# peach-xiao/EMRT

Measured on AMD Instinct MI355X. Metric: training tiles/sec at 256x256, higher is better.
Workload: dtype bf16; 1 GPU; EMRT ResNet50, Potsdam 256x256, 6 classes, batch 8 per GPU, fwd+bwd+SGD step (BASELINE configs[1]), bf16; global_batch=8, parallelism=dp1, hipgraph=True

## Files before the change

emrt_amd/csrc/common.hpp:

```cpp
#pragma once
#include <hip/hip_runtime.h>
#include <stdint.h>
#include <stdio.h>
#include <string.h>
#include "../../include/emrt_hip.h"

#define EMRT_F32 0
#define EMRT_BF16 1
#define EMRT_F16 2

namespace emrt {

extern thread_local char g_err[512];
inline int fail(const char* fn, const char* msg) {
  snprintf(g_err, sizeof(g_err), "%s: %s", fn, msg);
  return -1;
}
inline int check_launch(const char* fn) {
  hipError_t e = hipGetLastError();
  if (e != hipSuccess) {
    snprintf(g_err, sizeof(g_err), "%s: launch failed: %s", fn, hipGetErrorString(e));
    return -2;
  }
  return 0;
// ... 8 lines not shown
  int wgrad_split;
  int thin_cblk;
  int thin_blocks;
  int thin_ch;
  int no_thin_bwd;
  int igemm64_nst;
  int wgrad_nst;
  int pair_max;
  int msda_fwd_global;
  int msda_bwd_global;
  int msda_lds_min_pairs;
  int msda_bwd_dref_lds;
  int msda_band_halo;
  int msda_scatter_qsplit;
  int msda_scatter_cuts;
  int msda_fwd_chunks;
  int msda_fwd_threads;
  int msda_fwd_probe;
  int bn_block_kb;
  int bn_slice_c;
  int bn_operand_blocks;
  int ln_bwd_rows;
  int ln_bwd_max_blocks;
  int ln_bwd_threads;
  int ln_atomic;
  int gn_group_blocks;
  int gn_stat_rows;
  int gn_bwd_stat_rows;
  int gn_apply_rows;
  int igemm8p_probe;
  int igemm8p_cmajor;
  int igemm8p_min_blocks;
  int wgrad8p_min_steps;
  int wgrad8p_slab;
  int wgrad8p_xcd;
  int wgrad8p_force;
  int no_ksplit128;
  int wgrad_no_overwrite;
  int no_s2_dgrad;
  int wgroup_blocks;
  int wgroup_min_steps;
  int wgroup_max;
  int wgroup8;
  int wgroup8_blocks;
  int wgroup8_min_work;
  int msda_scatter_merge;
  int msda_scatter_mfma;
  int msda_mf_bands;
  int sgd_nt;
  int mha_bwd_split;
  int mha_valu;
  int no_bna;
  int memcpy_kernel;
  int xk;
};
extern Tuning g_tune;

struct Scratch {
  void* ptr; size_t bytes; void* stream;
  unsigned* tick;
  float* xk_part;
};
constexpr size_t SCRATCH_TICK_BYTES = 65536;
constexpr int SCRATCH_TICKS = (int)(SCRATCH_TICK_BYTES / 4);
constexpr size_t SCRATCH_XK_BYTES = 8u << 20;
extern Scratch g_scratch;

struct bf16_t {
  unsigned short v;
};
struct f16_t {
  unsigned short v;
};

__device__ __forceinline__ float to_f32(float x) { return x; }
__device__ __forceinline__ float to_f32(bf16_t x) { return __uint_as_float(((uint32_t)x.v) << 16); }
__device__ __forceinline__ float to_f32(f16_t x) { return (float)__builtin_bit_cast(_Float16, x.v); }
__device__ __forceinline__ float bf16_bits_to_f32(uint32_t lo16) { return __uint_as_float(lo16 << 16); }
__device__ __forceinline__ float f16_bits_to_f32(uint32_t lo16) { return (float)__builtin_bit_cast(_Float16, (unsigned short)lo16); }

template <class T>
__device__ __forceinline__ T from_f32(float f);
template <>
__device__ __forceinline__ float from_f32<float>(float f) {
  return f;
}
template <>
__device__ __forceinline__ bf16_t from_f32<bf16_t>(float f) {
  __bf16 b = (__bf16)f;
  bf16_t r;
  r.v = __builtin_bit_cast(unsigned short, b);
  return r;
}
template <>
__device__ __forceinline__ f16_t from_f32<f16_t>(float f) {
  f16_t r;
  r.v = __builtin_bit_cast(unsigned short, (_Float16)f);
  return r;
}
typedef __attribute__((ext_vector_type(2))) _Float16 emrt_half2_t;
typedef __attribute__((ext_vector_type(2))) float emrt_float2_t;
__device__ __forceinline__ uint32_t pack_f16x2(float lo, float hi) {
  emrt_half2_t h = __builtin_convertvector((emrt_float2_t){lo, hi}, emrt_half2_t);
  return __builtin_bit_cast(uint32_t, h);
}
__device__ __forceinline__ void unpack_f16x2(uint32_t w, float& lo, float& hi) {
// ... 249 lines not shown
```

emrt_amd/csrc/conv.hip:

```cpp
#include "common.hpp"
#include "bn_operand.hpp"
#include <stdlib.h>
#include <type_traits>

using namespace emrt;

typedef __attribute__((ext_vector_type(8))) __bf16 bf16x8_t;
typedef __attribute__((ext_vector_type(4))) short short4_t;
typedef __attribute__((ext_vector_type(16))) float f32x16_t;

struct ConvArgs {
  const void* in = nullptr;
  const void* w = nullptr;
  void* out = nullptr;
  const float* bias = nullptr;
  const float* scale = nullptr;
  const void* res = nullptr;
  int N = 0, H = 0, W = 0, C = 0, ldin = 0;
  long long in_bs = 0;
  int OH = 0, OW = 0, OC = 0, ldout = 0;
  long long out_bs = 0;
  int ldres = 0;
  long long res_bs = 0;
  int KH = 0, KW = 0, stride = 0, pad = 0;
// ... 1457 lines not shown
  const int gv = vec ? G : 1;
  const size_t lds = (size_t)gv * 2 * 2 * Cfg::BKM * Cfg::PITCH;
  static bool attr_done = false;
  if (!attr_done) {
    if (hipFuncSetAttribute(reinterpret_cast<const void*>(wgrad_kernel<T, true, G>), hipFuncAttributeMaxDynamicSharedMemorySize,
                            (int)((size_t)G * 4 * Cfg::BKM * Cfg::PITCH)) != hipSuccess ||
        hipFuncSetAttribute(reinterpret_cast<const void*>(wgrad_kernel<T, false, 1>), hipFuncAttributeMaxDynamicSharedMemorySize,
                            (int)((size_t)4 * Cfg::BKM * Cfg::PITCH)) != hipSuccess)
      return fail("emrt_conv2d_wgrad", "cannot raise the dynamic LDS limit");
    attr_done = true;
  }
  const int xcd = g_tune.wgrad8p_xcd;
  const unsigned grid1 = 8u * (unsigned)(((long long)tx * ty * S + 7) / 8);
  if (vec && g_tune.wgrad_nst == 3) {
    static bool attr3 = false;
    if (!attr3) { (void)hipFuncSetAttribute(reinterpret_cast<const void*>(wgrad_kernel<T, true, G, 3>), hipFuncAttributeMaxDynamicSharedMemorySize, (int)((size_t)G * 4 * Cfg::BKM * Cfg::PITCH)); attr3 = true; }
    hipLaunchKernelGGL((wgrad_kernel<T, true, G, 3>), dim3(grid1), dim3(256 * G), lds, st, a, tx, ty, S, xcd);
  } else if (vec) hipLaunchKernelGGL((wgrad_kernel<T, true, G>), dim3(grid1), dim3(256 * G), lds, st, a, tx, ty, S, xcd);
  else hipLaunchKernelGGL((wgrad_kernel<T, false, 1>), dim3(grid1), dim3(256), lds, st, a, tx, ty, S, xcd);
  return check_launch("emrt_conv2d_wgrad");
}

extern "C" int emrt_conv2d_wgrad(const void* x, const void* dy, float* dw,
                                 int N, int H, int W, int C, int ldx, long long x_bs,
                                 int OH, int OW, int OC, int lddy, long long dy_bs,
                                 int KH, int KW, int stride, int pad, float* dbias, int dilation, int dtype, void* stream) {
  EMRT_REQUIRE(x && dy && dw, "null pointer");
  const ConvShape s = {N, H, W, C, OH, OW, OC, KH, KW, stride, pad, dilation};
  EMRT_CONV_CHECK(s, ldx, x_bs, lddy, dy_bs, dtype, CK_DIMS);
  EMRT_REQUIRE(dilation >= 1, "bad dims");
  EMRT_CONV_CHECK(s, ldx, x_bs, lddy, dy_bs, dtype, CK_SIZE | CK_PIXELS);
  EMRT_REQUIRE_TRAIN_DTYPE(dtype);
  EMRT_CONV_CHECK(s, ldx, x_bs, lddy, dy_bs, dtype, CK_X | CK_Y | CK_X24);
  const WgradArgs a = wgrad_args(x, dy, dw, dbias, N, H, W, C, ldx, x_bs, OH, OW, OC, lddy, dy_bs, KH, KW, stride, pad, dilation, 0);
  hipStream_t st = (hipStream_t)stream;
  return with_train_dtype("emrt_conv2d_wgrad", dtype, [&](auto t) { return wgrad_dispatch<decltype(t)>(a, st); });
}

struct ThinBwdArgs {
  const void* x; const void* dy; const void* wd; void* dx; float* dw; float* dbias; double* stats; const void* mask_y;
  int HW, C, OC, ldx, lddy, lddx, ldy, accumulate, pix_per_block, cg_shift;
  float mask_scale;
  long long x_bs, dy_bs, dx_bs, y_bs, M;
  const float* bn_mean; const float* bn_invstd; const float* bn_gamma; const float* bn_beta;
};

template <class T, int CH>
struct VecN;
template <class T>
struct VecN<T, 4> : Vec4<T> {};
template <class T>
struct VecN<T, 8> : Vec8<T> {};

template <class T, int CH, int MASK, bool ACC, bool BNX = false>
__global__ __launch_bounds__(256, CH == 4 ? 4 : 2) void thin_bwd_kernel(ThinBwdArgs p) {
  constexpr int U = 2;
  using V = VecN<T, CH>;
  __shared__ float red[32 * 256];
  const T* x = (const T*)p.x;
  const T* dy = (const T*)p.dy;
  const T* wd = (const T*)p.wd;
  const T* ym = (const T*)p.mask_y;
  T* dx = (T*)p.dx;
  const int tid = threadIdx.x;
  const int CG = 1 << p.cg_shift, ppb = 256 >> p.cg_shift;
  const int cg = tid & (CG - 1), pl = tid >> p.cg_shift;
  const int c0 = (int)blockIdx.y * (CH << p.cg_shift) + cg * CH;
  const int lane = tid & 63;
  const int grp = CG < 64 ? CG : 64;
  const int gpos = lane & (grp - 1), gbase = lane - gpos;
  float w[8][CH], dwa[8][CH], ss[CH], sq[CH], db[8];
#pragma unroll
  for (int o = 0; o < 8; ++o) {
    db[o] = 0.f;
#pragma unroll
    for (int j = 0; j < CH; ++j) {
      w[o][j] = o < p.OC ? to_f32(wd[(c0 + j) * p.OC + o]) : 0.f;
      dwa[o][j] = 0.f;
    }
  }
#pragma unroll
  for (int j = 0; j < CH; ++j) { ss[j] = 0.f; sq[j] = 0.f; }
  float bsc[BNX ? CH : 1], bsh[BNX ? CH : 1];
  if (BNX) {
#pragma unroll
    for (int j = 0; j < CH; ++j) bn_scale_shift(p.bn_mean[c0 + j], p.bn_invstd[c0 + j], p.bn_gamma[c0 + j], p.bn_beta[c0 + j], bsc[j], bsh[j]);
  }
  const int xbs = (int)p.x_bs, dybs = (int)p.dy_bs, dxbs = (int)p.dx_bs, ybs = (int)p.y_bs, M = (int)p.M;
  const int m0 = (int)blockIdx.x * p.pix_per_block;
  const int m1 = m0 + p.pix_per_block < M ? m0 + p.pix_per_block : M;
  for (int mb = m0 + pl; mb < m1; mb += U * ppb) {
    float xv[U][CH], yv[U][CH], old[U][CH], mydy[U];
    bool ok[U];
    int oo[U];
#pragma unroll
    for (int u = 0; u < U; ++u) {
      const int m = mb + u * ppb;
      ok[u] = m < m1;
      mydy[u] = 0.f;
      if (!ok[u]) continue;
      const int nb = m / p.HW;
      const int pix = m - nb * p.HW;
      oo[u] = nb * dxbs + pix * p.lddx + c0;
      V::load(x + (nb * xbs + pix * p.ldx + c0), xv[u]);
      if (MASK == 2) V::load(ym + (nb * ybs + pix * p.ldy + c0), yv[u]);
      if (ACC) V::load(dx + oo[u], old[u]);
      if (gpos < p.OC) mydy[u] = to_f32(dy[nb * dybs + pix * p.lddy + gpos]);
    }
#pragma unroll
    for (int u = 0; u < U; ++u) {
      float dyv[8];
#pragma unroll
      for (int o = 0; o < 8; ++o) dyv[o] = __shfl(mydy[u], gbase + o, 64);
      if (!ok[u]) continue;
      if (BNX) {
#pragma unroll
        for (int j = 0; j < CH; ++j) xv[u][j] = fmaxf(fmaf(xv[u][j], bsc[j], bsh[j]), 0.f);
      }
      float v[CH];
#pragma unroll
      for (int j = 0; j < CH; ++j) {
        float a = 0.f;
#pragma unroll
        for (int o = 0; o < 8; ++o) a = fmaf(dyv[o], w[o][j], a);
        if (ACC) a += old[u][j];
        float second = 0.f;
        if (MASK) {
          second = MASK == 1 ? xv[u][j] : yv[u][j];
          a = second > 0.f ? a * p.mask_scale : 0.f;
        }
        v[j] = a;
        const float q = to_f32(from_f32<T>(a));
        ss[j] += q;
        sq[j] = fmaf(q, MASK ? second : q, sq[j]);
      }
      V::store(dx + oo[u], v);
#pragma unroll
      for (int o = 0; o < 8; ++o) {
#pragma unroll
        for (int j = 0; j < CH; ++j) dwa[o][j] = fmaf(dyv[o], xv[u][j], dwa[o][j]);
        if (cg == 0 && blockIdx.y == 0) db[o] += dyv[o];
      }
    }
  }
#pragma unroll
  for (int rnd = 0; rnd < CH / 4; ++rnd) {
    if (rnd * 32 >= p.OC * CH) break;
    if (rnd) __syncthreads();
#pragma unroll
    for (int k = 0; k < 32; ++k) red[k * 256 + tid] = dwa[(rnd * 32 + k) / CH][(rnd * 32 + k) % CH];
    __syncthreads();
    for (int k = pl; k < 32; k += ppb) {
      const int kk = rnd * 32 + k;
      if (kk >= p.OC * CH) break;
      float a = 0.f;
      for (int q = 0; q < ppb; ++q) a += red[k * 256 + q * CG + cg];
      atomicAdd(p.dw + (kk / CH) * p.C + c0 + (kk % CH), a);
    }
  }
  if (p.stats || p.dbias) {
    __syncthreads();
#pragma unroll
    for (int k = 0; k < CH; ++k) {
      red[k * 256 + tid] = ss[k];
      red[(CH + k) * 256 + tid] = sq[k];
    }
    if (cg == 0) {
#pragma unroll
      for (int k = 0; k < 8; ++k) red[(2 * CH + k) * 256 + pl] = db[k];
    }
    __syncthreads();
    if (p.stats) {
      double* rep = p.stats + (long long)(blockIdx.x & 7) * 2 * p.C;
      for (int k = pl; k < 2 * CH; k += ppb) {
        float a = 0.f;
        for (int q = 0; q < ppb; ++q) a += red[k * 256 + q * CG + cg];
        atomicAdd(rep + (k / CH) * p.C + c0 + (k % CH), (double)a);
      }
    }
    if (p.dbias && tid < p.OC) {
      float a = 0.f;
      for (int q = 0; q < ppb; ++q) a += red[(2 * CH + tid) * 256 + q];
      atomicAdd(p.dbias + tid, a);
    }
  }
}

template <class T>
static bool thin_bwd_ok(const ConvArgs& d, const WgradArgs& w) {
  constexpr int EPC = 4;
  const int C = w.C;
  if (w.KH != 1 || w.KW != 1 || w.stride != 1 || w.pad != 0 || w.OC > 8) return false;
  if (d.stat_x || (d.res && d.mask_y) || (d.res && d.res != d.out)) return false;
  if (C < 32 || C > 1024 || (C & (C - 1))) return false;
  const long long px = (long long)w.H * w.W - 1, LIM = 1ll << 31;
  if ((long long)w.N * w.H * w.W >= LIM || (w.N - 1) * w.x_bs + px * w.ldx + C >= LIM || (w.N - 1) * d.out_bs + px * d.ldout + C >= LIM ||
      (w.N - 1) * w.dy_bs + px * w.lddy + w.OC >= LIM || (d.mask_y && (w.N - 1) * d.y_bs + px * d.ldy + C >= LIM)) return false;
  auto al = [](const void* q) { return ((uintptr_t)q) % 16 == 0; };
  if (!al(w.x) || !al(d.out) || (d.mask_y && !al(d.mask_y))) return false;
  if (w.ldx % EPC || w.x_bs % EPC || d.ldout % EPC || d.out_bs % EPC) return false;
  if (d.mask_y && (d.ldy % EPC || d.y_bs % EPC)) return false;
  return true;
}

template <class T, int CH>
static int thin_bwd_launch_ch(const ConvArgs& d, const WgradArgs& w, hipStream_t st, const float* const* xbn = nullptr) {
  ThinBwdArgs a;
  a.x = w.x; a.dy = w.dy; a.wd = d.w; a.dx = d.out; a.dw = w.dw; a.dbias = w.dbias; a.stats = d.stats; a.mask_y = d.mask_y;
  a.HW = w.H * w.W; a.C = w.C; a.OC = w.OC; a.ldx = w.ldx; a.lddy = w.lddy; a.lddx = d.ldout; a.ldy = d.ldy;
  a.accumulate = d.res != nullptr;
  a.mask_scale = d.mask_scale;
  a.x_bs = w.x_bs; a.dy_bs = w.dy_bs; a.dx_bs = d.out_bs; a.y_bs = d.y_bs;
  a.M = (long long)w.N * w.H * w.W;
  int cblk = g_tune.thin_cblk;
  if (cblk < 8 * CH) cblk = 8 * CH;
  if (cblk > w.C) cblk = w.C;
  if (cblk > 256 * CH) cblk = 256 * CH;
  int sh = 0;
  while ((CH << sh) < cblk) ++sh;
  a.cg_shift = sh;
  const int cchunks = w.C / (CH << sh);
  const int ppb = 256 >> sh;
  const long long want_chunks = g_tune.thin_blocks > 0 ? g_tune.thin_blocks : 128;
  long long per = (a.M + want_chunks - 1) / want_chunks;
  per = (per + 2 * ppb - 1) / (2 * ppb) * (2 * ppb);
  if (per < 8 * ppb) per = 8 * ppb;
  a.pix_per_block = (int)per;
  const long long blocks = (a.M + per - 1) / per;
  const bool same = d.mask_y && d.mask_y == w.x && d.ldy == w.ldx && d.y_bs == w.x_bs;
  const int mask = !d.mask_y ? 0 : (same ? 1 : 2);
  const dim3 grid((unsigned)blocks, (unsigned)cchunks), block(256);
  a.bn_mean = a.bn_invstd = a.bn_gamma = a.bn_beta = nullptr;
  if (xbn) {
    if (mask != 1 || a.accumulate) return fail("emrt_bn_pointwise_bwd", "internal: the BatchNorm-operand form is the mask-from-input, overwrite form");
    a.bn_mean = xbn[0]; a.bn_invstd = xbn[1]; a.bn_gamma = xbn[2]; a.bn_beta = xbn[3];
    hipLaunchKernelGGL((thin_bwd_kernel<T, CH, 1, false, true>), grid, block, 0, st, a);
    return check_launch("emrt_bn_pointwise_bwd");
  }
  if (a.accumulate) {
    hipLaunchKernelGGL((thin_bwd_kernel<T, CH, 0, true>), grid, block, 0, st, a);
  } else if (mask == 0) {
    hipLaunchKernelGGL((thin_bwd_kernel<T, CH, 0, false>), grid, block, 0, st, a);
  } else if (mask == 1) {
    hipLaunchKernelGGL((thin_bwd_kernel<T, CH, 1, false>), grid, block, 0, st, a);
  } else {
    hipLaunchKernelGGL((thin_bwd_kernel<T, CH, 2, false>), grid, block, 0, st, a);
  }
  return check_launch("emrt_conv2d_bwd");
}

template <class T>
static int thin_bwd_launch(const ConvArgs& d, const WgradArgs& w, hipStream_t st, const float* const* xbn = nullptr) {
  const int want = g_tune.thin_ch;
  constexpr int EPC = 16 / (int)sizeof(T);
  const bool can8 = w.C >= 64 && w.ldx % 8 == 0 && w.x_bs % 8 == 0 && d.ldout % 8 == 0 && d.out_bs % 8 == 0 &&
                    (!d.mask_y || (d.ldy % 8 == 0 && d.y_bs % 8 == 0)) && EPC <= 8;
  if (want == 8 && can8) return thin_bwd_launch_ch<T, 8>(d, w, st, xbn);
  return thin_bwd_launch_ch<T, 4>(d, w, st, xbn);
}

struct ThinFwdArgs {
  const void* x; const void* w; const float* bias; void* out;
  int HW, C, OC, ldx, ldo;
  long long x_bs, o_bs, M;
};

template <class T>
struct Raw8;
template <>
struct Raw8<bf16_t> {
  uint4 q;
  __device__ __forceinline__ void load(const bf16_t* p) { q = *reinterpret_cast<const uint4*>(p); }
  __device__ __forceinline__ void unpack(float (&o)[8]) const { Vec8<bf16_t>::unpack(q, o); }
};
template <>
struct Raw8<float> {
  float4 a, b;
  __device__ __forceinline__ void load(const float* p) { a = *reinterpret_cast<const float4*>(p); b = *reinterpret_cast<const float4*>(p + 4); }
  __device__ __forceinline__ void unpack(float (&o)[8]) const { o[0] = a.x; o[1] = a.y; o[2] = a.z; o[3] = a.w; o[4] = b.x; o[5] = b.y; o[6] = b.z; o[7] = b.w; }
};

template <class T, int CGS>
__global__ __launch_bounds__(256, 2) void thin_fwd_bn_kernel(ThinFwdArgs p, BnOperand bn) {
  constexpr int CH = 8, U = 4;
  extern __shared__ float bn_lds[];
  const T* x = (const T*)p.x;
  const T* wp = (const T*)p.w;
  T* out = (T*)p.out;
  const int tid = threadIdx.x;
  constexpr int CG = 1 << CGS, ppb = 256 >> CGS;
  const int cg = tid & (CG - 1), pl = tid >> CGS;
  const int c0 = cg * CH;
  const int M = (int)p.M, HW = p.HW, xbs = (int)p.x_bs, obs = (int)p.o_bs;
  const int step = (int)gridDim.x * ppb * U;
  int mb = (int)blockIdx.x * ppb * U + pl;
  auto xoff = [&](int m) {
    const int mc = m < M ? m : 0;
    const int nb = mc / HW;
    return nb * xbs + (mc - nb * HW) * p.ldx + c0;
  };
  Raw8<T> xv[U], xn[U];
#pragma unroll
  for (int u = 0; u < U; ++u) xv[u].load(x + xoff(mb + u * ppb));
  bn_operand_preamble(bn, p.C, bn_lds, blockIdx.x == 0);
  float sc[CH], sh[CH], w[8][CH];
#pragma unroll
  for (int j = 0; j < CH; ++j) { sc[j] = bn_lds[c0 + j]; sh[j] = bn_lds[p.C + c0 + j]; }
#pragma unroll
  for (int o = 0; o < 8; ++o) {
    float wv[CH];
    Vec8<T>::load(wp + ((o < p.OC ? o : 0) * p.C + c0), wv);
#pragma unroll
    for (int j = 0; j < CH; ++j) w[o][j] = o < p.OC ? wv[j] : 0.f;
  }
  const float lo = bn.relu ? 0.f : -INFINITY;
  while (mb - pl < M) {
    const int mnext = mb + step;
#pragma unroll
    for (int u = 0; u < U; ++u) xn[u].load(x + xoff(mnext + u * ppb));
    float part[U * 8];
#pragma unroll
    for (int u = 0; u < U; ++u) {
      const bool ok = mb + u * ppb < M;
      float a[CH];
      xv[u].unpack(a);
#pragma unroll
      for (int j = 0; j < CH; ++j) a[j] = ok ? fmaxf(fmaf(a[j], sc[j], sh[j]), lo) : 0.f;
#pragma unroll
      for (int o = 0; o < 8; ++o) {
        float t = 0.f;
#pragma unroll
        for (int j = 0; j < CH; ++j) t = fmaf(a[j], w[o][j], t);
        part[u * 8 + o] = t;
// ... 493 lines not shown
```

emrt_amd/csrc/elementwise.hip:

```cpp
#include "common.hpp"
#include <stdlib.h>

using namespace emrt;

thread_local char emrt::g_err[512] = {0};

extern "C" const char* emrt_last_error(void) { return emrt::g_err; }
extern "C" int emrt_abi_version(void) { return 9; }

namespace {
struct TuneEntry { const char* name; int emrt::Tuning::*field; int def; };
const TuneEntry kTune[] = {
    {"conv_tile", &emrt::Tuning::conv_tile, 0},         {"wgrad_split", &emrt::Tuning::wgrad_split, 0},
    {"thin_cblk", &emrt::Tuning::thin_cblk, 64},        {"thin_blocks", &emrt::Tuning::thin_blocks, 128},
    {"thin_ch", &emrt::Tuning::thin_ch, 8},             {"no_thin_bwd", &emrt::Tuning::no_thin_bwd, 0},
    {"pair_max", &emrt::Tuning::pair_max, 768},         {"msda_fwd_global", &emrt::Tuning::msda_fwd_global, 0},
    {"bn_block_kb", &emrt::Tuning::bn_block_kb, 0},     {"ln_atomic", &emrt::Tuning::ln_atomic, 1},
    {"bn_slice_c", &emrt::Tuning::bn_slice_c, 0},
    {"msda_fwd_chunks", &emrt::Tuning::msda_fwd_chunks, 0}, {"msda_fwd_threads", &emrt::Tuning::msda_fwd_threads, 1024},
    {"msda_fwd_probe", &emrt::Tuning::msda_fwd_probe, 0}, {"wgrad_nst", &emrt::Tuning::wgrad_nst, 2},
    {"igemm64_nst", &emrt::Tuning::igemm64_nst, 3}, {"msda_bwd_global", &emrt::Tuning::msda_bwd_global, 0},
    {"msda_lds_min_pairs", &emrt::Tuning::msda_lds_min_pairs, 2048}, {"msda_bwd_dref_lds", &emrt::Tuning::msda_bwd_dref_lds, 1},
    {"gn_group_blocks", &emrt::Tuning::gn_group_blocks, 0}, {"gn_stat_rows", &emrt::Tuning::gn_stat_rows, 32},
    {"gn_bwd_stat_rows", &emrt::Tuning::gn_bwd_stat_rows, 32}, {"gn_apply_rows", &emrt::Tuning::gn_apply_rows, 8},
    {"msda_scatter_cuts", &emrt::Tuning::msda_scatter_cuts, 0}, {"msda_scatter_qsplit", &emrt::Tuning::msda_scatter_qsplit, 0}, {"msda_band_halo", &emrt::Tuning::msda_band_halo, 0},
    {"igemm8p_probe", &emrt::Tuning::igemm8p_probe, 0}, {"igemm8p_min_blocks", &emrt::Tuning::igemm8p_min_blocks, 160}, {"igemm8p_cmajor", &emrt::Tuning::igemm8p_cmajor, 0},
    {"wgrad8p_min_steps", &emrt::Tuning::wgrad8p_min_steps, 8}, {"wgrad8p_slab", &emrt::Tuning::wgrad8p_slab, 1}, {"wgrad8p_force", &emrt::Tuning::wgrad8p_force, 0}, {"wgrad8p_xcd", &emrt::Tuning::wgrad8p_xcd, 1},
    {"wgrad_no_overwrite", &emrt::Tuning::wgrad_no_overwrite, 0}, {"no_ksplit128", &emrt::Tuning::no_ksplit128, 0}, {"ln_bwd_rows", &emrt::Tuning::ln_bwd_rows, 0}, {"ln_bwd_max_blocks", &emrt::Tuning::ln_bwd_max_blocks, 0}, {"bn_operand_blocks", &emrt::Tuning::bn_operand_blocks, 0}, {"no_s2_dgrad", &emrt::Tuning::no_s2_dgrad, 0}, {"wgroup_blocks", &emrt::Tuning::wgroup_blocks, 1024}, {"wgroup_min_steps", &emrt::Tuning::wgroup_min_steps, 32}, {"wgroup_max", &emrt::Tuning::wgroup_max, 0},
    {"no_bna", &emrt::Tuning::no_bna, 0}, {"memcpy_kernel", &emrt::Tuning::memcpy_kernel, 0}, {"xk", &emrt::Tuning::xk, 0}, {"mha_valu", &emrt::Tuning::mha_valu, 0}, {"mha_bwd_split", &emrt::Tuning::mha_bwd_split, 1}, {"msda_scatter_merge", &emrt::Tuning::msda_scatter_merge, 0},
    {"wgroup8", &emrt::Tuning::wgroup8, 0}, {"wgroup8_blocks", &emrt::Tuning::wgroup8_blocks, 0}, {"wgroup8_min_work", &emrt::Tuning::wgroup8_min_work, 6000},
    {"msda_scatter_mfma", &emrt::Tuning::msda_scatter_mfma, 1}, {"sgd_nt", &emrt::Tuning::sgd_nt, 1}, {"ln_bwd_threads", &emrt::Tuning::ln_bwd_threads, 512}, {"msda_mf_bands", &emrt::Tuning::msda_mf_bands, 0},
};
emrt::Tuning tuning_from_env() {
  emrt::Tuning t;
  for (const TuneEntry& e : kTune) {
    char env[64] = "EMRT_";
    size_t n = strlen(env);
    for (const char* c = e.name; *c && n + 1 < sizeof(env); ++c) env[n++] = (char)((*c >= 'a' && *c <= 'z') ? *c - 32 : *c);
    env[n] = 0;
    const char* v = (strcmp(e.name, "msda_fwd_probe") == 0 || strcmp(e.name, "igemm8p_probe") == 0) ? nullptr : getenv(env);
    t.*(e.field) = v ? atoi(v) : e.def;
  }
  return t;
}
}
emrt::Tuning emrt::g_tune = tuning_from_env();
emrt::Scratch emrt::g_scratch = {nullptr, 0, nullptr, nullptr, nullptr};

extern "C" int emrt_set_scratch(void* ptr, size_t bytes, void* stream) {
  EMRT_REQUIRE((ptr != nullptr) == (bytes > 0) && ((uintptr_t)ptr) % 256 == 0, "scratch must be 256-byte aligned device memory (or nullptr, 0)");
  if (ptr && ptr == emrt::g_scratch.ptr && emrt::g_scratch.tick && bytes == emrt::g_scratch.bytes + emrt::SCRATCH_TICK_BYTES + emrt::SCRATCH_XK_BYTES) {
    emrt::g_scratch.stream = stream;
    return 0;
  }
  emrt::g_scratch.ptr = ptr;
  emrt::g_scratch.bytes = bytes;
  emrt::g_scratch.stream = stream;
  emrt::g_scratch.tick = nullptr;
  emrt::g_scratch.xk_part = nullptr;
  if (ptr && bytes >= (16u << 20) + emrt::SCRATCH_XK_BYTES + emrt::SCRATCH_TICK_BYTES && bytes % 256 == 0) {
    emrt::g_scratch.bytes = bytes - emrt::SCRATCH_TICK_BYTES - emrt::SCRATCH_XK_BYTES;
    emrt::g_scratch.xk_part = reinterpret_cast<float*>(static_cast<char*>(ptr) + emrt::g_scratch.bytes);
    emrt::g_scratch.tick = reinterpret_cast<unsigned*>(static_cast<char*>(ptr) + emrt::g_scratch.bytes + emrt::SCRATCH_XK_BYTES);
    if (hipMemsetAsync(emrt::g_scratch.tick, 0, emrt::SCRATCH_TICK_BYTES, (hipStream_t)stream) != hipSuccess) {
      emrt::g_scratch.tick = nullptr;
      return emrt::fail("emrt_set_scratch", "cannot zero the arrival counters");
    }
  }
  return 0;
}

// ... 411 lines not shown
```

emrt_amd/csrc/norm.hip:

```cpp
#include "common.hpp"
#include "bn_operand.hpp"
#include <stdlib.h>

using namespace emrt;

template <class T, int MODE>
__global__ __launch_bounds__(256) void col_reduce_kernel(const T* __restrict__ x, int ldx, const T* __restrict__ dy, int lddy,
                                                         const T* __restrict__ y, int ldy, const float* __restrict__ mean,
                                                         const float* __restrict__ invstd, long long M, int C, int tx_n,
                                                         float* __restrict__ partial, long long rpb, long long bs,
                                                         double* __restrict__ dsums, float* __restrict__ facc,
                                                         const float* __restrict__ mgamma = nullptr, const float* __restrict__ mbeta = nullptr) {
  __shared__ float red[256 * 8];
  const int ty_n = 256 / tx_n;
  const int tx = threadIdx.x % tx_n, ty = threadIdx.x / tx_n;
  const int c = (blockIdx.y * tx_n + tx) * 4;
  float s0[4] = {0, 0, 0, 0}, s1[4] = {0, 0, 0, 0};
  if (c < C) {
    float mu[4] = {0, 0, 0, 0}, is[4] = {1, 1, 1, 1};
    float msc[MODE == 3 ? 4 : 1], msh[MODE == 3 ? 4 : 1];
    if (MODE == 1 || MODE == 3) {
#pragma unroll
      for (int e = 0; e < 4; ++e) { mu[e] = mean[c + e]; is[e] = invstd[c + e]; }
      if constexpr (MODE == 3) {
#pragma unroll
        for (int e = 0; e < 4; ++e) bn_scale_shift(mu[e], is[e], mgamma[c + e], mbeta[c + e], msc[e], msh[e]);
      }
    }
    for (long long r = (long long)blockIdx.x * ty_n + ty; r < M; r += (long long)gridDim.x * ty_n) {
      float v[4];
      if (MODE == 0) {
        Vec4<T>::load(x + r * ldx + c, v);
#pragma unroll
        for (int e = 0; e < 4; ++e) { s0[e] += v[e]; s1[e] = fmaf(v[e], v[e], s1[e]); }
      } else if (MODE == 1 || MODE == 3) {
        const long long rs = (long long)gridDim.x * ty_n;
        float vv[4][4], gg[4][4], oo[4][4];
#pragma unroll
        for (int u = 0; u < 4; ++u) {
          const long long ru = r + u * rs < M ? r + u * rs : r;
          Vec4<T>::load(x + ru * ldx + c, vv[u]);
          Vec4<T>::load(dy + ru * lddy + c, gg[u]);
          if (y) Vec4<T>::load(y + ru * ldy + c, oo[u]);
        }
#pragma unroll
        for (int u = 0; u < 4; ++u) {
          const bool ok = r + u * rs < M;
#pragma unroll
          for (int e = 0; e < 4; ++e) {
            float g = ok ? gg[u][e] : 0.f;
            if (y) g = oo[u][e] > 0.f ? g : 0.f;
            if constexpr (MODE == 3) g = fmaf(vv[u][e], msc[e], msh[e]) > 0.f ? g : 0.f;
            s0[e] += g;
            s1[e] = fmaf(g, (vv[u][e] - mu[e]) * is[e], s1[e]);
          }
        }
        r += 3 * rs;
      } else {
        const long long bb = (M | rpb) <= 0xffffffffll ? (long long)((unsigned)r / (unsigned)rpb) : r / rpb;
        Vec4<T>::load(x + bb * bs + (r - bb * rpb) * ldx + c, v);
#pragma unroll
        for (int e = 0; e < 4; ++e) s0[e] += v[e];
      }
    }
  }
#pragma unroll
  for (int e = 0; e < 4; ++e) { red[threadIdx.x * 8 + e] = s0[e]; red[threadIdx.x * 8 + 4 + e] = s1[e]; }
  __syncthreads();
  if (ty == 0 && c < C) {
    for (int t = 1; t < ty_n; ++t) {
#pragma unroll
      for (int e = 0; e < 4; ++e) { s0[e] += red[(t * tx_n + tx) * 8 + e]; s1[e] += red[(t * tx_n + tx) * 8 + 4 + e]; }
    }
    if (dsums) {
      double* rep = dsums + (long long)(blockIdx.x & 7) * 2 * C;
#pragma unroll
      for (int e = 0; e < 4; ++e) { atomicAdd(rep + c + e, (double)s0[e]); atomicAdd(rep + C + c + e, (double)s1[e]); }
    } else if (facc) {
#pragma unroll
      for (int e = 0; e < 4; ++e)
        if (c + e < C) atomicAdd(facc + c + e, s0[e]);
    } else {
      float* pp = partial + (long long)blockIdx.x * 2 * C;
#pragma unroll
      for (int e = 0; e < 4; ++e) { pp[c + e] = s0[e]; pp[C + c + e] = s1[e]; }
    }
  }
}

static inline void col_reduce_geometry(long long M, int C, int& tx_n, int& gx, int& gy) {
  int quads = (C + 3) / 4;
  tx_n = 64;
  while (tx_n > 1 && tx_n / 2 >= quads) tx_n /= 2;
  gy = (quads + tx_n - 1) / tx_n;
  int ty_n = 256 / tx_n;
  long long want = (M + (long long)ty_n * 8 - 1) / ((long long)ty_n * 8);
  long long cap = 512 / gy;
  if (cap < 1) cap = 1;
  gx = (int)(want < 1 ? 1 : (want > cap ? cap : want));
}

__global__ __launch_bounds__(256) void bn_sum_partials_kernel(const float* __restrict__ partial, int nblk, int C, float* __restrict__ sums ) {
  __shared__ double red[8][33];
  const int cx = threadIdx.x & 31, py = threadIdx.x >> 5;
  const int c = blockIdx.x * 32 + cx;
  double s = 0.0;
  if (c < 2 * C)
    for (int b = py; b < nblk; b += 8) s += (double)partial[(long long)b * 2 * C + c];
  red[py][cx] = s;
  __syncthreads();
  if (py == 0 && c < 2 * C) {
    double t = 0.0;
#pragma unroll
    for (int k = 0; k < 8; ++k) t += red[k][cx];
    sums[c] = (float)t;
  }
}

__global__ __launch_bounds__(256) void partials_acc_kernel(const float* __restrict__ partial, int nblk, int C, float* __restrict__ dgamma,
                                                          float* __restrict__ dbeta) {
  __shared__ double red[8][33];
  const int cx = threadIdx.x & 31, py = threadIdx.x >> 5;
  const int c = blockIdx.x * 32 + cx;
  double s = 0.0;
  if (c < 2 * C)
    for (int b = py; b < nblk; b += 8) s += (double)partial[(long long)b * 2 * C + c];
  red[py][cx] = s;
  __syncthreads();
  if (py == 0 && c < 2 * C) {
    double t = 0.0;
#pragma unroll
    for (int k = 0; k < 8; ++k) t += red[k][cx];
    if (c < C) { if (dbeta) dbeta[c] += (float)t; }
    else if (dgamma) dgamma[c - C] += (float)t;
  }
}

__global__ void bn_bwd_finalize_kernel(const float* __restrict__ sums, int C, float* __restrict__ dgamma, float* __restrict__ dbeta) {
  const int c = blockIdx.x * blockDim.x + threadIdx.x;
  if (c >= C) return;
  if (dbeta) dbeta[c] += sums[c];
  if (dgamma) dgamma[c] += sums[C + c];
}

template <class T, bool JOIN = false>
__global__ __launch_bounds__(512) void bn_apply_kernel(const T* __restrict__ x, int ldx, const T* __restrict__ res, int ldres,
                                                       T* __restrict__ y, int ldy, const double* __restrict__ sums, double inv_count,
                                                       float eps, float momentum, float* __restrict__ mean_out,
                                                       float* __restrict__ invstd_out, float* __restrict__ run_mean,
                                                       float* __restrict__ run_var, const float* __restrict__ gamma,
// ... 1065 lines not shown
                                  float* r_invstd, float* r_run_mean, float* r_run_var, const float* r_gamma, const float* r_beta, long long M,
                                  int C, int relu, int dtype, void* stream) {
  EMRT_REQUIRE_TRAIN_DTYPE(dtype);
  EMRT_REQUIRE(x && res_raw && y && gamma && beta && sums && mean && invstd, "null pointer");
  EMRT_REQUIRE(r_sums && r_mean && r_invstd && r_gamma && r_beta && r_count > 0.0 && count > 0.0 && (r_run_mean != nullptr) == (r_run_var != nullptr),
               "the shortcut's BatchNorm needs sums, mean, invstd, gamma, beta and a positive count");
  EMRT_REQUIRE(C % 4 == 0 && ldx % 4 == 0 && ldy % 4 == 0 && ldres % 4 == 0, "C and ld must be multiples of 4");
  int threads, rpp, cs;
  dim3 grid;
  EMRT_REQUIRE(bn_rowgeom(M, C, threads, rpp, cs, grid), "unsupported channel count (C/4 must divide 256, or C <= 2048)");
  BnOperand r;
  r.sums = r_sums; r.inv_count = 1.0 / r_count; r.eps = r_eps; r.momentum = r_momentum; r.mean = r_mean; r.invstd = r_invstd;
  r.run_mean = r_run_mean; r.run_var = r_run_var; r.gamma = r_gamma; r.beta = r_beta; r.relu = 0;
  hipStream_t st = (hipStream_t)stream;
  const double inv_count = 1.0 / count;
  const size_t lds = (size_t)4 * cs * sizeof(float);
  return with_train_dtype("emrt_bn_apply_join", dtype, [&](auto t) {
    using T = decltype(t);
    hipLaunchKernelGGL((bn_apply_kernel<T, true>), grid, dim3(threads), lds, st, (const T*)x, ldx, (const T*)res_raw, ldres, (T*)y, ldy, sums, inv_count, eps, momentum, mean, invstd, run_mean, run_var, gamma, beta, M, C, relu, rpp, cs, r);
    return check_launch("emrt_bn_apply_join");
  });
}

__global__ __launch_bounds__(256) void bn_fold_kernel(const float* __restrict__ params, const float* __restrict__ buffers,
                                                      const long long* __restrict__ desc, float eps, float* __restrict__ out) {
  const long long* d = desc + 7 * (long long)blockIdx.x;
  const float* gamma = params + d[0];
  const float* beta = params + d[1];
  const float* mean = buffers + d[2];
  const float* var = buffers + d[3];
  const int C = (int)d[4];
  float* o = out + d[5];
  const float* cbias = d[6] >= 0 ? params + d[6] : nullptr;
  for (int c = threadIdx.x; c < C; c += blockDim.x) {
    const float sc = gamma[c] * rsqrtf(var[c] + eps);
    o[c] = sc;
    o[C + c] = beta[c] + ((cbias ? cbias[c] : 0.f) - mean[c]) * sc;
  }
}
extern "C" int emrt_bn_fold(const float* params, const float* buffers, const long long* desc, int n, float eps, float* out, void* stream) {
  EMRT_REQUIRE(params && buffers && desc && out && n > 0, "null pointer");
  hipLaunchKernelGGL(bn_fold_kernel, dim3(n), dim3(256), 0, (hipStream_t)stream, params, buffers, desc, eps, out);
  return check_launch("emrt_bn_fold");
}

extern "C" int emrt_bn_bwd_reduce(const void* x, int ldx, const void* dy, int lddy, const void* y, int ldy, const float* mean,
                                  const float* invstd, long long M, int C, double* sums, const float* mask_gamma, const float* mask_beta,
                                  int dtype, void* stream) {
  EMRT_REQUIRE_TRAIN_DTYPE(dtype);
  EMRT_REQUIRE(x && dy && mean && invstd && sums, "null pointer");
  EMRT_REQUIRE((mask_gamma != nullptr) == (mask_beta != nullptr) && !(mask_beta && y), "mask_gamma and mask_beta come together and replace y");
  EMRT_REQUIRE(C % 4 == 0 && ldx % 4 == 0 && lddy % 4 == 0 && (!y || ldy % 4 == 0), "C and ld must be multiples of 4");
  int tx, gx, gy;
  col_reduce_geometry(M, C, tx, gx, gy);
  hipStream_t st = (hipStream_t)stream;
  return with_train_dtype("emrt_bn_bwd_reduce", dtype, [&](auto t) {
    using T = decltype(t);
    if (mask_beta) {
      hipLaunchKernelGGL((col_reduce_kernel<T, 3>), dim3(gx, gy), dim3(256), 0, st, (const T*)x, ldx, (const T*)dy, lddy, (const T*)nullptr, 0, mean, invstd, M, C, tx, nullptr, M, 0LL, sums, nullptr, mask_gamma, mask_beta);
      return check_launch("emrt_bn_bwd_reduce");
    }
    hipLaunchKernelGGL((col_reduce_kernel<T, 1>), dim3(gx, gy), dim3(256), 0, st, (const T*)x, ldx, (const T*)dy, lddy, (const T*)y, ldy, mean, invstd, M, C, tx, nullptr, M, 0LL, sums, nullptr);
    return check_launch("emrt_bn_bwd_reduce");
  });
}

extern "C" int emrt_bn_bwd_dx(const void* x, int ldx, const void* dy, int lddy, const void* y, int ldy, void* dx, int lddx,
                              void* dres, int lddres, const float* mean, const float* invstd, const float* gamma,
                              const double* sums, const double* local_sums, double count, float* dgamma, float* dbeta, long long M,
                              int C, const float* beta_y_moments, int sums_vs_x, const float* mask_beta, int dtype, void* stream) {
  EMRT_REQUIRE_TRAIN_DTYPE(dtype);
  EMRT_REQUIRE(x && dy && dx && mean && invstd && gamma && sums, "null pointer");
  EMRT_REQUIRE(!(mask_beta && (y || beta_y_moments || sums_vs_x)), "mask_beta (ReLU mask re-derived from x) excludes y and the fused-sum forms");
  EMRT_REQUIRE(C % 4 == 0 && ldx % 4 == 0 && lddy % 4 == 0 && lddx % 4 == 0, "C and ld must be multiples of 4");
  int threads, rpp, cs;
  dim3 grid;
  EMRT_REQUIRE(bn_rowgeom(M, C, threads, rpp, cs, grid), "unsupported channel count (C/4 must divide 256, or C <= 2048)");
  hipStream_t st = (hipStream_t)stream;
  return with_train_dtype("emrt_bn_bwd_dx", dtype, [&](auto t) {
    using T = decltype(t);
    if (mask_beta) {
      hipLaunchKernelGGL((bn_bwd_dx_kernel<T, true>), grid, dim3(threads), (size_t)2 * cs * sizeof(float), st, (const T*)x, ldx, (const T*)dy, lddy, (const T*)nullptr, 0, (T*)dx, lddx, (T*)dres, lddres, mean, invstd, gamma, sums, local_sums, 1.0 / count, dgamma, dbeta, M, C, rpp, cs, nullptr, 0, mask_beta);
      return check_launch("emrt_bn_bwd_dx");
    }
    hipLaunchKernelGGL((bn_bwd_dx_kernel<T>), grid, dim3(threads), (size_t)2 * cs * sizeof(float), st, (const T*)x, ldx, (const T*)dy, lddy, (const T*)y, ldy, (T*)dx, lddx, (T*)dres, lddres, mean, invstd, gamma, sums, local_sums, 1.0 / count, dgamma, dbeta, M, C, rpp, cs, beta_y_moments, sums_vs_x, mask_beta);
    return check_launch("emrt_bn_bwd_dx");
  });
}

template <class T>
__global__ __launch_bounds__(256) void colsum_scalar_kernel(const T* __restrict__ x, int ldx, long long rpb, long long bs, long long M,
                                                            float* __restrict__ dbias) {
  __shared__ float red[4];
  const int c = blockIdx.x;
  float s = 0.f;
  for (long long r = threadIdx.x; r < M; r += 256) {
    const long long bb = r / rpb;
    s += to_f32(x[bb * bs + (r - bb * rpb) * ldx + c]);
  }
  s = wave_sum(s);
  if ((threadIdx.x & 63) == 0) red[threadIdx.x >> 6] = s;
  __syncthreads();
  if (threadIdx.x == 0) dbias[c] += red[0] + red[1] + red[2] + red[3];
}

extern "C" int emrt_colsum_acc(const void* x, int ldx, long long rows_per_batch, long long x_bs, long long M, int C, float* dbias,
                               void* workspace, int dtype, void* stream) {
  EMRT_REQUIRE_TRAIN_DTYPE(dtype);
  EMRT_REQUIRE(rows_per_batch > 0, "bad batch geometry");
  EMRT_REQUIRE(x && dbias && workspace, "null pointer");
  return with_train_dtype("emrt_colsum_acc", dtype, [&](auto t) {
    using T = decltype(t);
    if (C % 4 != 0 || ldx % 4 != 0 || x_bs % 4 != 0) {
      hipStream_t st0 = (hipStream_t)stream;
      hipLaunchKernelGGL((colsum_scalar_kernel<T>), dim3(C), dim3(256), 0, st0, (const T*)x, ldx, rows_per_batch, x_bs, M, dbias);
// ... 483 lines not shown
```

Baseline: 1036 tiles/s.

## Software-prefetch loads in thin conv backward and BN backward reduce kernels

Adds register-level software pipelining to two memory-bound backward kernels. The thin 1x1 conv backward kernel keeps UP pixels of raw x and dy loads in flight, issuing the next rows' loads before computing on the current ones. The BN backward column reduce prefetches NS rows of x and dy ahead and halves the block cap so each thread streams more rows. This is meant to hide global-memory latency, at the cost of more registers and possible occupancy loss. It is gated by a new stream_geom tuning knob that defaults to on.

```diff
diff --git a/emrt_amd/csrc/common.hpp b/emrt_amd/csrc/common.hpp
--- a/emrt_amd/csrc/common.hpp
+++ b/emrt_amd/csrc/common.hpp
@@ -84,6 +84,7 @@
   int mha_valu;
   int no_bna;
   int memcpy_kernel;
+  int stream_geom;
   int xk;
 };
 extern Tuning g_tune;
diff --git a/emrt_amd/csrc/conv.hip b/emrt_amd/csrc/conv.hip
--- a/emrt_amd/csrc/conv.hip
+++ b/emrt_amd/csrc/conv.hip
@@ -1533,9 +1533,40 @@
 template <class T>
 struct VecN<T, 8> : Vec8<T> {};
 
-template <class T, int CH, int MASK, bool ACC, bool BNX = false>
+template <class T, int CH>
+struct RawN;
+template <>
+struct RawN<bf16_t, 8> {
+  uint4 q;
+  __device__ __forceinline__ void load(const bf16_t* p) { q = *reinterpret_cast<const uint4*>(p); }
+  __device__ __forceinline__ void unpack(float (&o)[8]) const { Vec8<bf16_t>::unpack(q, o); }
+};
+template <>
+struct RawN<bf16_t, 4> {
+  uint2 q;
+  __device__ __forceinline__ void load(const bf16_t* p) { q = *reinterpret_cast<const uint2*>(p); }
+  __device__ __forceinline__ void unpack(float (&o)[4]) const {
+    o[0] = bf16_bits_to_f32(q.x & 0xffffu); o[1] = __uint_as_float(q.x & 0xffff0000u);
+    o[2] = bf16_bits_to_f32(q.y & 0xffffu); o[3] = __uint_as_float(q.y & 0xffff0000u);
+  }
+};
+template <int CH>
+struct RawN<float, CH> {
+  float4 a[CH / 4];
+  __device__ __forceinline__ void load(const float* p) {
+#pragma unroll
+    for (int i = 0; i < CH / 4; ++i) a[i] = *reinterpret_cast<const float4*>(p + 4 * i);
+  }
+  __device__ __forceinline__ void unpack(float (&o)[CH]) const {
+#pragma unroll
+    for (int i = 0; i < CH / 4; ++i) { o[4 * i] = a[i].x; o[4 * i + 1] = a[i].y; o[4 * i + 2] = a[i].z; o[4 * i + 3] = a[i].w; }
+  }
+};
+
+template <class T, int CH, int MASK, bool ACC, bool BNX = false, int PF = 0>
 __global__ __launch_bounds__(256, CH == 4 ? 4 : 2) void thin_bwd_kernel(ThinBwdArgs p) {
   constexpr int U = 2;
+  constexpr int UP = sizeof(T) == 2 ? 4 : 2;
   using V = VecN<T, CH>;
   __shared__ float red[32 * 256];
   const T* x = (const T*)p.x;
@@ -1550,13 +1581,38 @@
   const int lane = tid & 63;
   const int grp = CG < 64 ? CG : 64;
   const int gpos = lane & (grp - 1), gbase = lane - gpos;
+  const int xbs = (int)p.x_bs, dybs = (int)p.dy_bs, dxbs = (int)p.dx_bs, ybs = (int)p.y_bs, M = (int)p.M;
+  const int m0 = (int)blockIdx.x * p.pix_per_block;
+  const int m1 = m0 + p.pix_per_block < M ? m0 + p.pix_per_block : M;
+  RawN<T, CH> sx[PF ? UP : 1];
+  T sdy[PF ? UP : 1];
+  int so[PF ? UP : 1];
+  const int dlane = gpos < p.OC ? gpos : 0;
+  auto fill = [&](int u, int m) {
+    const bool has = m < m1;
+    const int mc = has ? m : m0;
+    const int nb = mc / p.HW;
+    const int pix = mc - nb * p.HW;
+    so[u] = has ? nb * dxbs + pix * p.lddx + c0 : -1;
+    sx[u].load(x + (nb * xbs + pix * p.ldx + c0));
+    sdy[u] = dy[nb * dybs + pix * p.lddy + dlane];
+  };
+  if constexpr (PF != 0) {
+#pragma unroll
+    for (int u = 0; u < UP; ++u) fill(u, m0 + pl + u * ppb);
+  }
   float w[8][CH], dwa[8][CH], ss[CH], sq[CH], db[8];
 #pragma unroll
   for (int o = 0; o < 8; ++o) {
     db[o] = 0.f;
 #pragma unroll
     for (int j = 0; j < CH; ++j) {
-      w[o][j] = o < p.OC ? to_f32(wd[(c0 + j) * p.OC + o]) : 0.f;
+      if constexpr (PF != 0) {
+        const float wv = to_f32(wd[(c0 + j) * p.OC + (o < p.OC ? o : 0)]);
+        w[o][j] = o < p.OC ? wv : 0.f;
+      } else {
+        w[o][j] = o < p.OC ? to_f32(wd[(c0 + j) * p.OC + o]) : 0.f;
+      }
       dwa[o][j] = 0.f;
     }
   }
@@ -1567,61 +1623,80 @@
 #pragma unroll
     for (int j = 0; j < CH; ++j) bn_scale_shift(p.bn_mean[c0 + j], p.bn_invstd[c0 + j], p.bn_gamma[c0 + j], p.bn_beta[c0 + j], bsc[j], bsh[j]);
   }
-  const int xbs = (int)p.x_bs, dybs = (int)p.dy_bs, dxbs = (int)p.dx_bs, ybs = (int)p.y_bs, M = (int)p.M;
-  const int m0 = (int)blockIdx.x * p.pix_per_block;
-  const int m1 = m0 + p.pix_per_block < M ? m0 + p.pix_per_block : M;
-  for (int mb = m0 + pl; mb < m1; mb += U * ppb) {
-    float xv[U][CH], yv[U][CH], old[U][CH], mydy[U];
-    bool ok[U];
-    int oo[U];
-#pragma unroll
-    for (int u = 0; u < U; ++u) {
-      const int m = mb + u * ppb;
-      ok[u] = m < m1;
-      mydy[u] = 0.f;
-      if (!ok[u]) continue;
-      const int nb = m / p.HW;
-      const int pix = m - nb * p.HW;
-      oo[u] = nb * dxbs + pix * p.lddx + c0;
-      V::load(x + (nb * xbs + pix * p.ldx + c0), xv[u]);
-      if (MASK == 2) V::load(ym + (nb * ybs + pix * p.ldy + c0), yv[u]);
-      if (ACC) V::load(dx + oo[u], old[u]);
-      if (gpos < p.OC) mydy[u] = to_f32(dy[nb * dybs + pix * p.lddy + gpos]);
-    }
-#pragma unroll
-    for (int u = 0; u < U; ++u) {
-      float dyv[8];
-#pragma unroll
-      for (int o = 0; o < 8; ++o) dyv[o] = __shfl(mydy[u], gbase + o, 64);
-      if (!ok[u]) continue;
-      if (BNX) {
-#pragma unroll
-        for (int j = 0; j < CH; ++j) xv[u][j] = fmaxf(fmaf(xv[u][j], bsc[j], bsh[j]), 0.f);
-      }
-      float v[CH];
-#pragma unroll
-      for (int j = 0; j < CH; ++j) {
-        float a = 0.f;
-#pragma unroll
-        for (int o = 0; o < 8; ++o) a = fmaf(dyv[o], w[o][j], a);
-        if (ACC) a += old[u][j];
-        float second = 0.f;
-        if (MASK) {
-          second = MASK == 1 ? xv[u][j] : yv[u][j];
-          a = second > 0.f ? a * p.mask_scale : 0.f;
-        }
-        v[j] = a;
-        const float q = to_f32(from_f32<T>(a));
-        ss[j] += q;
-        sq[j] = fmaf(q, MASK ? second : q, sq[j]);
-      }
-      V::store(dx + oo[u], v);
-#pragma unroll
-      for (int o = 0; o < 8; ++o) {
-#pragma unroll
-        for (int j = 0; j < CH; ++j) dwa[o][j] = fmaf(dyv[o], xv[u][j], dwa[o][j]);
-        if (cg == 0 && blockIdx.y == 0) db[o] += dyv[o];
-      }
+  auto pixel = [&](float (&xa)[CH], const float (&ya)[CH], const float (&olda)[CH], float dyu, bool live, int off) {
+    float dyv[8];
+#pragma unroll
+    for (int o = 0; o < 8; ++o) dyv[o] = __shfl(dyu, gbase + o, 64);
+    if (!live) return;
+    if (BNX) {
+#pragma unroll
+      for (int j = 0; j < CH; ++j) xa[j] = fmaxf(fmaf(xa[j], bsc[j], bsh[j]), 0.f);
+    }
+    float v[CH];
+#pragma unroll
+    for (int j = 0; j < CH; ++j) {
+      float a = 0.f;
+#pragma unroll
+      for (int o = 0; o < 8; ++o) a = fmaf(dyv[o], w[o][j], a);
+      if (ACC) a += olda[j];
+      float second = 0.f;
+      if (MASK) {
+        second = MASK == 1 ? xa[j] : ya[j];
+        a = second > 0.f ? a * p.mask_scale : 0.f;
+      }
+      v[j] = a;
+      const float q = to_f32(from_f32<T>(a));
+      ss[j] += q;
+      sq[j] = fmaf(q, MASK ? second : q, sq[j]);
+    }
+    V::store(dx + off, v);
+#pragma unroll
+    for (int o = 0; o < 8; ++o) {
+#pragma unroll
+      for (int j = 0; j < CH; ++j) dwa[o][j] = fmaf(dyv[o], xa[j], dwa[o][j]);
+      if (cg == 0 && blockIdx.y == 0) db[o] += dyv[o];
+    }
+  };
+  if constexpr (PF != 0) {
+    for (int mb = m0 + pl; mb < m1; mb += UP * ppb) {
+#pragma unroll
+      for (int u = 0; u < UP; ++u) {
+        const int m = mb + u * ppb;
+        const int off = so[u];
+        const bool live = off >= 0;
+        const float dyu = live && gpos < p.OC ? to_f32(sdy[u]) : 0.f;
+        float xa[CH], ya[CH], olda[CH];
+        sx[u].unpack(xa);
+        if (live) {
+          if (MASK == 2) { const int nb = m / p.HW; V::load(ym + (nb * ybs + (m - nb * p.HW) * p.ldy + c0), ya); }
+          if (ACC) V::load(dx + off, olda);
+        }
+        fill(u, m + UP * ppb);
+        pixel(xa, ya, olda, dyu, live, off);
+      }
+    }
+  } else {
+    for (int mb = m0 + pl; mb < m1; mb += U * ppb) {
+      float xv[U][CH], yv[U][CH], old[U][CH], mydy[U];
+      bool ok[U];
+      int oo[U];
+#pragma unroll
+      for (int u = 0; u < U; ++u) {
+        const int m = mb + u * ppb;
+        ok[u] = m < m1;
+        mydy[u] = 0.f;
+        oo[u] = 0;
+        if (!ok[u]) continue;
+        const int nb = m / p.HW;
+        const int pix = m - nb * p.HW;
+        oo[u] = nb * dxbs + pix * p.lddx + c0;
+        V::load(x + (nb * xbs + pix * p.ldx + c0), xv[u]);
+        if (MASK == 2) V::load(ym + (nb * ybs + pix * p.ldy + c0), yv[u]);
+        if (ACC) V::load(dx + oo[u], old[u]);
+        if (gpos < p.OC) mydy[u] = to_f32(dy[nb * dybs + pix * p.lddy + gpos]);
+      }
+#pragma unroll
+      for (int u = 0; u < U; ++u) pixel(xv[u], yv[u], old[u], mydy[u], ok[u], oo[u]);
     }
   }
 #pragma unroll
@@ -1712,20 +1787,26 @@
   const int mask = !d.mask_y ? 0 : (same ? 1 : 2);
   const dim3 grid((unsigned)blocks, (unsigned)cchunks), block(256);
   a.bn_mean = a.bn_invstd = a.bn_gamma = a.bn_beta = nullptr;
+  constexpr bool can_pf = CH == 8;
+  const bool pf = can_pf && g_tune.stream_geom != 1 && !a.accumulate;
   if (xbn) {
     if (mask != 1 || a.accumulate) return fail("emrt_bn_pointwise_bwd", "internal: the BatchNorm-operand form is the mask-from-input, overwrite form");
     a.bn_mean = xbn[0]; a.bn_invstd = xbn[1]; a.bn_gamma = xbn[2]; a.bn_beta = xbn[3];
-    hipLaunchKernelGGL((thin_bwd_kernel<T, CH, 1, false, true>), grid, block, 0, st, a);
+    if (pf) hipLaunchKernelGGL((thin_bwd_kernel<T, CH, 1, false, true, can_pf ? 1 : 0>), grid, block, 0, st, a);
+    else hipLaunchKernelGGL((thin_bwd_kernel<T, CH, 1, false, true>), grid, block, 0, st, a);
     return check_launch("emrt_bn_pointwise_bwd");
   }
   if (a.accumulate) {
     hipLaunchKernelGGL((thin_bwd_kernel<T, CH, 0, true>), grid, block, 0, st, a);
   } else if (mask == 0) {
-    hipLaunchKernelGGL((thin_bwd_kernel<T, CH, 0, false>), grid, block, 0, st, a);
+    if (pf) hipLaunchKernelGGL((thin_bwd_kernel<T, CH, 0, false, false, can_pf ? 1 : 0>), grid, block, 0, st, a);
+    else hipLaunchKernelGGL((thin_bwd_kernel<T, CH, 0, false>), grid, block, 0, st, a);
   } else if (mask == 1) {
-    hipLaunchKernelGGL((thin_bwd_kernel<T, CH, 1, false>), grid, block, 0, st, a);
+    if (pf) hipLaunchKernelGGL((thin_bwd_kernel<T, CH, 1, false, false, can_pf ? 1 : 0>), grid, block, 0, st, a);
+    else hipLaunchKernelGGL((thin_bwd_kernel<T, CH, 1, false>), grid, block, 0, st, a);
   } else {
-    hipLaunchKernelGGL((thin_bwd_kernel<T, CH, 2, false>), grid, block, 0, st, a);
+    if (pf) hipLaunchKernelGGL((thin_bwd_kernel<T, CH, 2, false, false, can_pf ? 1 : 0>), grid, block, 0, st, a);
+    else hipLaunchKernelGGL((thin_bwd_kernel<T, CH, 2, false>), grid, block, 0, st, a);
   }
   return check_launch("emrt_conv2d_bwd");
 }
@@ -1747,19 +1828,7 @@
 };
 
 template <class T>
-struct Raw8;
-template <>
-struct Raw8<bf16_t> {
-  uint4 q;
-  __device__ __forceinline__ void load(const bf16_t* p) { q = *reinterpret_cast<const uint4*>(p); }
-  __device__ __forceinline__ void unpack(float (&o)[8]) const { Vec8<bf16_t>::unpack(q, o); }
-};
-template <>
-struct Raw8<float> {
-  float4 a, b;
-  __device__ __forceinline__ void load(const float* p) { a = *reinterpret_cast<const float4*>(p); b = *reinterpret_cast<const float4*>(p + 4); }
-  __device__ __forceinline__ void unpack(float (&o)[8]) const { o[0] = a.x; o[1] = a.y; o[2] = a.z; o[3] = a.w; o[4] = b.x; o[5] = b.y; o[6] = b.z; o[7] = b.w; }
-};
+using Raw8 = RawN<T, 8>;
 
 template <class T, int CGS>
 __global__ __launch_bounds__(256, 2) void thin_fwd_bn_kernel(ThinFwdArgs p, BnOperand bn) {
diff --git a/emrt_amd/csrc/elementwise.hip b/emrt_amd/csrc/elementwise.hip
--- a/emrt_amd/csrc/elementwise.hip
+++ b/emrt_amd/csrc/elementwise.hip
@@ -16,7 +16,7 @@
     {"thin_ch", &emrt::Tuning::thin_ch, 8},             {"no_thin_bwd", &emrt::Tuning::no_thin_bwd, 0},
     {"pair_max", &emrt::Tuning::pair_max, 768},         {"msda_fwd_global", &emrt::Tuning::msda_fwd_global, 0},
     {"bn_block_kb", &emrt::Tuning::bn_block_kb, 0},     {"ln_atomic", &emrt::Tuning::ln_atomic, 1},
-    {"bn_slice_c", &emrt::Tuning::bn_slice_c, 0},
+    {"bn_slice_c", &emrt::Tuning::bn_slice_c, 0},       {"stream_geom", &emrt::Tuning::stream_geom, 0},
     {"msda_fwd_chunks", &emrt::Tuning::msda_fwd_chunks, 0}, {"msda_fwd_threads", &emrt::Tuning::msda_fwd_threads, 1024},
     {"msda_fwd_probe", &emrt::Tuning::msda_fwd_probe, 0}, {"wgrad_nst", &emrt::Tuning::wgrad_nst, 2},
     {"igemm64_nst", &emrt::Tuning::igemm64_nst, 3}, {"msda_bwd_global", &emrt::Tuning::msda_bwd_global, 0},
diff --git a/emrt_amd/csrc/norm.hip b/emrt_amd/csrc/norm.hip
--- a/emrt_amd/csrc/norm.hip
+++ b/emrt_amd/csrc/norm.hip
@@ -4,7 +4,23 @@
 
 using namespace emrt;
 
-template <class T, int MODE>
+template <class T>
+struct Raw4 {
+  float4 q;
+  __device__ __forceinline__ void load(const float* p) { q = *reinterpret_cast<const float4*>(p); }
+  __device__ __forceinline__ void unpack(float (&o)[4]) const { o[0] = q.x; o[1] = q.y; o[2] = q.z; o[3] = q.w; }
+};
+template <>
+struct Raw4<bf16_t> {
+  uint2 q;
+  __device__ __forceinline__ void load(const bf16_t* p) { q = *reinterpret_cast<const uint2*>(p); }
+  __device__ __forceinline__ void unpack(float (&o)[4]) const {
+    o[0] = bf16_bits_to_f32(q.x & 0xffffu); o[1] = __uint_as_float(q.x & 0xffff0000u);
+    o[2] = bf16_bits_to_f32(q.y & 0xffffu); o[3] = __uint_as_float(q.y & 0xffff0000u);
+  }
+};
+
+template <class T, int MODE, int PF = 0>
 __global__ __launch_bounds__(256) void col_reduce_kernel(const T* __restrict__ x, int ldx, const T* __restrict__ dy, int lddy,
                                                          const T* __restrict__ y, int ldy, const float* __restrict__ mean,
                                                          const float* __restrict__ invstd, long long M, int C, int tx_n,
@@ -16,7 +32,56 @@
   const int tx = threadIdx.x % tx_n, ty = threadIdx.x / tx_n;
   const int c = (blockIdx.y * tx_n + tx) * 4;
   float s0[4] = {0, 0, 0, 0}, s1[4] = {0, 0, 0, 0};
-  if (c < C) {
+  if constexpr (PF != 0 && (MODE == 1 || MODE == 3)) {
+    constexpr int NS = sizeof(T) == 2 ? 4 : 2;
+    long long r = (long long)blockIdx.x * ty_n + ty;
+    if (c < C && r < M) {
+      const long long rs = (long long)gridDim.x * ty_n;
+      Raw4<T> sx[NS], sg[NS];
+      auto fill = [&](int u, long long rr) {
+        sx[u].load(x + rr * ldx + c);
+        sg[u].load(dy + rr * lddy + c);
+      };
+#pragma unroll
+      for (int u = 0; u < NS; ++u) fill(u, r + u * rs < M ? r + u * rs : r);
+      float mu[4], is[4], msc[MODE == 3 ? 4 : 1], msh[MODE == 3 ? 4 : 1];
+#pragma unroll
+      for (int e = 0; e < 4; ++e) { mu[e] = mean[c + e]; is[e] = invstd[c + e]; }
+      if constexpr (MODE == 3) {
+#pragma unroll
+        for (int e = 0; e < 4; ++e) bn_scale_shift(mu[e], is[e], mgamma[c + e], mbeta[c + e], msc[e], msh[e]);
+      }
+      float a0[2][4] = {{0, 0, 0, 0}, {0, 0, 0, 0}}, a1[2][4] = {{0, 0, 0, 0}, {0, 0, 0, 0}};
+      auto sum_slot = [&](int u, const Raw4<T>& kx, const Raw4<T>& kg, bool ok) {
+        float vv[4], gg[4];
+        kx.unpack(vv);
+        kg.unpack(gg);
+#pragma unroll
+        for (int e = 0; e < 4; ++e) {
+          float g = ok ? gg[e] : 0.f;
+          if constexpr (MODE == 3) g = fmaf(vv[e], msc[e], msh[e]) > 0.f ? g : 0.f;
+          a0[u & 1][e] += g;
+          a1[u & 1][e] = fmaf(g, (vv[e] - mu[e]) * is[e], a1[u & 1][e]);
+        }
+      };
+      for (; r < M; r += NS * rs) {
+        if (r + NS * rs < M) {
+#pragma unroll
+          for (int u = 0; u < NS; ++u) {
+            const long long rn = r + u * rs + NS * rs;
+            const Raw4<T> kx = sx[u], kg = sg[u];
+            fill(u, rn < M ? rn : r);
+            sum_slot(u, kx, kg, true);
+          }
+        } else {
+#pragma unroll
+          for (int u = 0; u < NS; ++u) sum_slot(u, sx[u], sg[u], r + u * rs < M);
+        }
+      }
+#pragma unroll
+      for (int e = 0; e < 4; ++e) { s0[e] = a0[0][e] + a0[1][e]; s1[e] = a1[0][e] + a1[1][e]; }
+    }
+  } else if (c < C) {
     float mu[4] = {0, 0, 0, 0}, is[4] = {1, 1, 1, 1};
     float msc[MODE == 3 ? 4 : 1], msh[MODE == 3 ? 4 : 1];
     if (MODE == 1 || MODE == 3) {
@@ -88,14 +153,14 @@
   }
 }
 
-static inline void col_reduce_geometry(long long M, int C, int& tx_n, int& gx, int& gy) {
+static inline void col_reduce_geometry(long long M, int C, int& tx_n, int& gx, int& gy, int max_blocks = 512) {
   int quads = (C + 3) / 4;
   tx_n = 64;
   while (tx_n > 1 && tx_n / 2 >= quads) tx_n /= 2;
   gy = (quads + tx_n - 1) / tx_n;
   int ty_n = 256 / tx_n;
   long long want = (M + (long long)ty_n * 8 - 1) / ((long long)ty_n * 8);
-  long long cap = 512 / gy;
+  long long cap = max_blocks / gy;
   if (cap < 1) cap = 1;
   gx = (int)(want < 1 ? 1 : (want > cap ? cap : want));
 }
@@ -1267,15 +1332,19 @@
   EMRT_REQUIRE((mask_gamma != nullptr) == (mask_beta != nullptr) && !(mask_beta && y), "mask_gamma and mask_beta come together and replace y");
   EMRT_REQUIRE(C % 4 == 0 && ldx % 4 == 0 && lddy % 4 == 0 && (!y || ldy % 4 == 0), "C and ld must be multiples of 4");
   int tx, gx, gy;
-  col_reduce_geometry(M, C, tx, gx, gy);
+  const bool pf = g_tune.stream_geom != 1 && !y;
+  col_reduce_geometry(M, C, tx, gx, gy, pf ? 256 : 512);
   hipStream_t st = (hipStream_t)stream;
   return with_train_dtype("emrt_bn_bwd_reduce", dtype, [&](auto t) {
     using T = decltype(t);
+    const dim3 grid(gx, gy), block(256);
     if (mask_beta) {
-      hipLaunchKernelGGL((col_reduce_kernel<T, 3>), dim3(gx, gy), dim3(256), 0, st, (const T*)x, ldx, (const T*)dy, lddy, (const T*)nullptr, 0, mean, invstd, M, C, tx, nullptr, M, 0LL, sums, nullptr, mask_gamma, mask_beta);
+      if (pf) hipLaunchKernelGGL((col_reduce_kernel<T, 3, 1>), grid, block, 0, st, (const T*)x, ldx, (const T*)dy, lddy, (const T*)nullptr, 0, mean, invstd, M, C, tx, nullptr, M, 0LL, sums, nullptr, mask_gamma, mask_beta);
+      else hipLaunchKernelGGL((col_reduce_kernel<T, 3>), grid, block, 0, st, (const T*)x, ldx, (const T*)dy, lddy, (const T*)nullptr, 0, mean, invstd, M, C, tx, nullptr, M, 0LL, sums, nullptr, mask_gamma, mask_beta);
       return check_launch("emrt_bn_bwd_reduce");
     }
-    hipLaunchKernelGGL((col_reduce_kernel<T, 1>), dim3(gx, gy), dim3(256), 0, st, (const T*)x, ldx, (const T*)dy, lddy, (const T*)y, ldy, mean, invstd, M, C, tx, nullptr, M, 0LL, sums, nullptr);
+    if (pf) hipLaunchKernelGGL((col_reduce_kernel<T, 1, 1>), grid, block, 0, st, (const T*)x, ldx, (const T*)dy, lddy, (const T*)y, ldy, mean, invstd, M, C, tx, nullptr, M, 0LL, sums, nullptr, nullptr, nullptr);
+    else hipLaunchKernelGGL((col_reduce_kernel<T, 1>), grid, block, 0, st, (const T*)x, ldx, (const T*)dy, lddy, (const T*)y, ldy, mean, invstd, M, C, tx, nullptr, M, 0LL, sums, nullptr);
     return check_launch("emrt_bn_bwd_reduce");
   });
 }
```

Measured after the change: 1041 tiles/s, median of 6. Within noise of the previous version (+0.4%).
